# SerCharles/CN-RMA

Hardware: AMD Instinct MI355X
Metric: scenes/sec fwd (40-view->192^3 voxel): dense unprojection + RMA + voxelise + FCAF3D + decode (higher is better)
Workload: dtype f32 (sparse conv f16x3: 22-bit operands, fp32 accumulate; value_f32_conv = exact fp32); 1 GPU; NS: 40 views x 256 ch x 480x640 fp32 maps (channels_last) -> grid 192x192x192, N=300, max_points=500000, FCAF3D MinkResNet34 + head, 1 HIP graph per scene, 3 in flight; M_rows=72216505, M_selected=500000, M_unique=496819

## Files before the change

### cn-rma_amd/csrc/common.h

```cpp
#pragma once
#include <hip/hip_runtime.h>
#include <stdint.h>

#include "../../include/cnrma.h"

#define CNRMA_LAUNCH_CHECK()                      \
  do {                                            \
    hipError_t e__ = hipGetLastError();           \
    if (e__ != hipSuccess) return -(int)e__;      \
  } while (0)

static inline hipStream_t as_stream(void* s) { return reinterpret_cast<hipStream_t>(s); }
static inline int64_t ceil_div(int64_t a, int64_t b) { return (a + b - 1) / b; }

template <int UNUSED = 0>
__global__ __launch_bounds__(256) void cnrma_fill_kernel(uint32_t* __restrict__ p, uint32_t word, size_t n_words) {
  const size_t n4 = (((uintptr_t)p & 15) == 0) ? n_words / 4 : 0;
  const uint4 w4 = make_uint4(word, word, word, word);
  for (size_t i = (size_t)blockIdx.x * blockDim.x + threadIdx.x; i < n4; i += (size_t)gridDim.x * blockDim.x)
    reinterpret_cast<uint4*>(p)[i] = w4;
  for (size_t i = 4 * n4 + (size_t)blockIdx.x * blockDim.x + threadIdx.x; i < n_words; i += (size_t)gridDim.x * blockDim.x)
    p[i] = word;
}
static inline hipError_t cnrma_fill_bytes(void* p, int byte, size_t n_bytes, hipStream_t st) {
  if (n_bytes == 0) return hipSuccess;
  if ((n_bytes & 3) != 0 || ((uintptr_t)p & 3) != 0) return hipMemsetAsync(p, byte, n_bytes, st);
  const uint32_t b = (uint32_t)(byte & 0xFF), word = b | (b << 8) | (b << 16) | (b << 24);
  size_t blocks = (n_bytes / 16 + 255) / 256;
  blocks = blocks < 1 ? 1 : (blocks > 2048 ? 2048 : blocks);
  hipLaunchKernelGGL(cnrma_fill_kernel<0>, dim3((unsigned)blocks), dim3(256), 0, st, reinterpret_cast<uint32_t*>(p), word,
                     n_bytes / 4);
  return hipGetLastError();
}
// ... 139 lines not shown
```

### cn-rma_amd/csrc/sparse.hip

```cpp
#include <cstdio>
#include <type_traits>
#include "common.h"

#include <hipcub/hipcub.hpp>

namespace {

struct UniqueWs {
  int32_t* slot;
  int32_t* idx;
  uint8_t* flag;
  void* scan;
  uint64_t* key_a; uint64_t* key_b;
  int32_t* val_a; int32_t* val_b;
  void* sort_tmp; size_t sort_tmp_bytes;
  int32_t* range_err;
};

size_t sort_temp_bytes(int64_t n) {
  size_t bytes = 0;
  hipError_t e = hipcub::DeviceRadixSort::SortPairs(nullptr, bytes, (const uint64_t*)nullptr, (uint64_t*)nullptr,
                                                    (const int32_t*)nullptr, (int32_t*)nullptr, (int)n, 0, 64, nullptr);
  if (e != hipSuccess || bytes == 0) bytes = (size_t)n * 16 + (1u << 20);
  (void)hipGetLastError();
// ... 3275 lines not shown
                                               int64_t no_cap, int precleared, void* stream) {
  if (n_cap <= 0 || no_cap <= 0 || in_stride <= 0 || kernel_size < 1 || kernel_size > 3) return CNRMA_EINVAL;
  const int K = kernel_size * kernel_size * kernel_size;
  hipStream_t st = as_stream(stream);
  if (!precleared) {
    hipError_t e = cnrma_fill_bytes(nbr, 0xFF, (size_t)no_cap * K * sizeof(int32_t), st);
    if (e != hipSuccess) return -(int)e;
  }
  hipLaunchKernelGGL(kernel_map_strided_kernel, dim3((unsigned)ceil_div(n_cap, 256)), dim3(256), 0, st, in_coords,
                     n_cap, n_dev, in_stride, kernel_size, out_hash_keys, out_hash_vals, hash_cap, nbr);
  CNRMA_LAUNCH_CHECK();
  return 0;
}

extern "C" size_t cnrma_sparse_conv_workspace_bytes(int64_t no_cap, int Cout, int K) {
  if (K <= 1 || no_cap >= 65536) return 0;
  return (size_t)K * (size_t)no_cap * (size_t)Cout * sizeof(float);
}

#ifdef CNRMA_EXPERIMENTS
extern "C" int cnrma_debug_conv_tuning(const int* v, int n) {
  ConvTune t;
  int* f[] = {&t.shape, &t.splits, &t.pf, &t.ablate, &t.ws, &t.xcd, &t.go, &t.nb};
  if (n < 0 || n > 8 || (n > 0 && v == nullptr)) return CNRMA_EINVAL;
  for (int i = 0; i < n; ++i) *f[i] = v[i];
  g_conv_tune = t;
  return 0;
}
#endif

extern "C" int cnrma_sparse_conv_plan(int64_t no_cap, int Cin, int Cout, int K, int mode, int slices, size_t workspace_bytes,
                                      int* out6) {
  if (out6 == nullptr || Cin <= 0 || Cout <= 0 || K <= 0 || K > 27 || no_cap <= 0 || mode < 0 || mode > 3) return CNRMA_EINVAL;
  const bool six = mode != 0 && Cin % 32 == 0;
  const ConvMode m = mode == 3 ? CONV_EXACT : static_cast<ConvMode>(mode);
  const ConvPlan pl = plan_conv(no_cap, Cin, Cout, K, m, six, slices > 1 ? slices : 1, workspace_bytes > 0, workspace_bytes);
  out6[0] = pl.bm; out6[1] = pl.bn; out6[2] = pl.splits; out6[3] = pl.k_per_split; out6[4] = pl.pf; out6[5] = pl.shape;
  return 0;
}

extern "C" int cnrma_sparse_conv_f32(const float* in_feats, int Cin, const int32_t* nbr, int K, const float* weight,
                                     int Cout, const float* scale, const float* shift, const float* residual, int act,
                                     float* out_feats, int64_t no_cap, const int32_t* no_dev, void* workspace,
                                     size_t workspace_bytes, void* stream) {
  ConvArgs p = conv_args(in_feats, Cin, nbr, K, Cout, out_feats, no_cap, no_dev, workspace);
  p.weight = weight;
  return launch_conv(with_epilogue(p, scale, shift, residual, act), CONV_EXACT, nullptr, workspace_bytes, as_stream(stream));
}
// ... 977 lines not shown
```

### cn-rma_amd/csrc/util.hip

```cpp
#include "common.h"

extern "C" int cnrma_abi_version(void) { return CNRMA_ABI_VERSION; }

extern "C" int cnrma_fill_bytes_u8(void* dst, int byte, size_t n_bytes, void* stream) {
  if (dst == nullptr || (n_bytes & 3) != 0 || (reinterpret_cast<uintptr_t>(dst) & 3) != 0) return CNRMA_EINVAL;
  if (n_bytes == 0) return 0;
  const hipError_t e = cnrma_fill_bytes(dst, byte, n_bytes, reinterpret_cast<hipStream_t>(stream));
  return e == hipSuccess ? 0 : -(int)e;
}

__global__ __launch_bounds__(256) void range_violations_kernel(const int32_t* __restrict__ v, const int32_t* __restrict__ lo,
                                                               const int32_t* __restrict__ hi, int n, int32_t* __restrict__ out) {
  __shared__ int sm[4];
  int c = 0;
  for (int i = threadIdx.x; i < n; i += 256) c += (v[i] < lo[i] || v[i] > hi[i]) ? 1 : 0;
  for (int o = 32; o > 0; o >>= 1) c += __shfl_down(c, o, 64);
  if ((threadIdx.x & 63) == 0) sm[threadIdx.x >> 6] = c;
  __syncthreads();
  if (threadIdx.x == 0) out[0] = sm[0] + sm[1] + sm[2] + sm[3];
}

extern "C" int cnrma_range_violations_i32(const int32_t* values, const int32_t* lo, const int32_t* hi, int n, int32_t* out,
                                          void* stream) {
  if (values == nullptr || lo == nullptr || hi == nullptr || out == nullptr || n <= 0 || n > 4096) return CNRMA_EINVAL;
  hipLaunchKernelGGL(range_violations_kernel, dim3(1), dim3(256), 0, reinterpret_cast<hipStream_t>(stream), values, lo, hi, n, out);
  CNRMA_LAUNCH_CHECK();
  return 0;
}

namespace {

constexpr int SCAN_BLOCK = 256;
constexpr int SCAN_VECS = 4;
constexpr int SCAN_ITEMS = 4 * SCAN_VECS;
constexpr int SCAN_TILE = SCAN_BLOCK * SCAN_ITEMS;
constexpr int SCAN_WAVE_ITEMS = 64 * SCAN_ITEMS;

template <typename T>
__device__ __forceinline__ int scan_load(const T* in, int64_t i, int64_t n) {
  return i < n ? (int)in[i] : 0;
}

__device__ __forceinline__ int64_t scan_vec_base(int64_t tile_base, int k) {
  return tile_base + (int64_t)(threadIdx.x >> 6) * SCAN_WAVE_ITEMS + (int64_t)(k * 64 + (threadIdx.x & 63)) * 4;
}

template <typename T>
__device__ __forceinline__ void scan_load_vec(const T* __restrict__ in, int64_t i, int64_t n, bool wide, int v[4]) {
  static_assert(sizeof(T) == 4 || sizeof(T) == 1, "int32 items or byte masks");
  if (wide) {
    if constexpr (sizeof(T) == 4) {
      const int4 q = *reinterpret_cast<const int4*>(in + i);
      v[0] = q.x; v[1] = q.y; v[2] = q.z; v[3] = q.w;
    } else {
      const uint32_t q = *reinterpret_cast<const uint32_t*>(in + i);
      v[0] = (int)(q & 255u); v[1] = (int)((q >> 8) & 255u); v[2] = (int)((q >> 16) & 255u); v[3] = (int)(q >> 24);
    }
  } else {
#pragma unroll
    for (int j = 0; j < 4; ++j) v[j] = scan_load(in, i + j, n);
  }
}

template <typename T>
__global__ __launch_bounds__(SCAN_BLOCK) void scan_tile_sums(const T* __restrict__ in, int32_t* __restrict__ tile_sum,
                                                             int64_t n, int aligned) {
  __shared__ int smem[SCAN_BLOCK / 64 + 1];
  const int64_t tile_base = (int64_t)blockIdx.x * SCAN_TILE;
  const bool wide = aligned != 0 && tile_base + SCAN_TILE <= n;
  int s = 0;
#pragma unroll
  for (int k = 0; k < SCAN_VECS; ++k) {
    int v[4];
    scan_load_vec(in, scan_vec_base(tile_base, k), n, wide, v);
    s += (v[0] + v[1]) + (v[2] + v[3]);
  }
  int total;
  block_excl_scan<SCAN_BLOCK>(s, smem, &total);
  if (threadIdx.x == 0) tile_sum[blockIdx.x] = total;
}

__global__ __launch_bounds__(1024) void scan_tile_offsets(int32_t* __restrict__ tile_sum, int64_t n_tiles) {
  __shared__ int smem[1024 / 64 + 1];
  const int64_t per = (n_tiles + 1023) / 1024;
  const int64_t lo = (int64_t)threadIdx.x * per;
  const int64_t hi = lo + per < n_tiles ? lo + per : n_tiles;
  int s = 0;
  for (int64_t i = lo; i < hi; ++i) s += tile_sum[i];
  int total;
  int run = block_excl_scan<1024>(s, smem, &total);
  for (int64_t i = lo; i < hi; ++i) {
    const int v = tile_sum[i];
    tile_sum[i] = run;
    run += v;
  }
  if (threadIdx.x == 0) tile_sum[n_tiles] = total;
}

template <typename T, int MODE, bool OWN_OFFSET>
__global__ __launch_bounds__(SCAN_BLOCK) void scan_apply(const T* __restrict__ in, const int32_t* __restrict__ tile_off,
                                                         int32_t* __restrict__ out, int32_t* __restrict__ total_out,
                                                         int64_t n, int64_t n_tiles, int aligned) {
  __shared__ int smem[SCAN_BLOCK / 64 + 1];
  __shared__ int wave_sum[SCAN_BLOCK / 64];
  const int64_t tile_base = (int64_t)blockIdx.x * SCAN_TILE;
  const bool wide = aligned != 0 && tile_base + SCAN_TILE <= n;
  const int lane = threadIdx.x & 63, wid = threadIdx.x >> 6;
  int v[SCAN_VECS][4];
  int ex[SCAN_VECS];
  int run = 0;
#pragma unroll
  for (int k = 0; k < SCAN_VECS; ++k) {
    scan_load_vec(in, scan_vec_base(tile_base, k), n, wide, v[k]);
    const int q = (v[k][0] + v[k][1]) + (v[k][2] + v[k][3]);
    const int incl = wave_incl_scan(q);
    ex[k] = run + incl - q;
    run += __shfl(incl, 63, 64);
  }
  if (lane == 0) wave_sum[wid] = run;
  int offset, grand = 0;
  if constexpr (OWN_OFFSET) {
    const int upto = blockIdx.x == 0 ? (int)n_tiles : (int)blockIdx.x;
    int part = 0;
    for (int i = threadIdx.x; i < upto; i += SCAN_BLOCK) part += tile_off[i];
    int sum;
    block_excl_scan<SCAN_BLOCK>(part, smem, &sum);
    offset = blockIdx.x == 0 ? 0 : sum;
// ... 12 lines not shown
    int at = offset + ex[k];
#pragma unroll
    for (int j = 0; j < 4; ++j) {
      r[j] = (MODE == 0) ? at : (v[k][j] ? at : -1);
      at += v[k][j];
    }
    if (wide) {
      *reinterpret_cast<int4*>(out + i) = make_int4(r[0], r[1], r[2], r[3]);
    } else {
#pragma unroll
      for (int j = 0; j < 4; ++j)
        if (i + j < n) out[i + j] = r[j];
    }
  }
  if (blockIdx.x == 0 && threadIdx.x == 0) {
    if (MODE == 0) out[n] = grand;
    if (total_out) total_out[0] = grand;
  }
}

constexpr int SCAN_SINGLE_MAX = 32768;
template <typename T, int MODE>
__global__ __launch_bounds__(1024) void scan_single_kernel(const T* __restrict__ in, int32_t* __restrict__ out,
                                                           int32_t* __restrict__ total_out, int n) {
  __shared__ int smem[1024 / 64 + 1];
  const int per = (n + 1023) / 1024;
  const int lo = threadIdx.x * per, hi = min(lo + per, n);
  int s = 0;
  for (int i = lo; i < hi; ++i) s += (int)in[i];
  int total;
  int run = block_excl_scan<1024>(s, smem, &total);
  for (int i = lo; i < hi; ++i) {
    const int v = (int)in[i];
    out[i] = (MODE == 0) ? run : (v ? run : -1);
    run += v;
  }
  if (threadIdx.x == 0) {
    if (MODE == 0) out[n] = total;
    if (total_out) total_out[0] = total;
  }
}

template <typename T, int MODE>
int run_scan(const T* in, int32_t* out, int32_t* total_out, int64_t n, void* workspace, hipStream_t st) {
  if (n < 0) return CNRMA_EINVAL;
  if (n <= SCAN_SINGLE_MAX) {
    hipLaunchKernelGGL((scan_single_kernel<T, MODE>), dim3(1), dim3(1024), 0, st, in, out, total_out, (int)n);
    CNRMA_LAUNCH_CHECK();
    return 0;
  }
  int64_t n_tiles = ceil_div(n > 0 ? n : 1, SCAN_TILE);
  int32_t* tile = reinterpret_cast<int32_t*>(workspace);
  const int aligned = (reinterpret_cast<uintptr_t>(out) & 15) == 0 && (reinterpret_cast<uintptr_t>(in) & (4 * sizeof(T) - 1)) == 0;
  hipLaunchKernelGGL((scan_tile_sums<T>), dim3((unsigned)n_tiles), dim3(SCAN_BLOCK), 0, st, in, tile, n, aligned);
  if (n_tiles <= SCAN_TILE) {
    hipLaunchKernelGGL((scan_apply<T, MODE, true>), dim3((unsigned)n_tiles), dim3(SCAN_BLOCK), 0, st, in, tile, out, total_out,
                       n, n_tiles, aligned);
  } else {
    hipLaunchKernelGGL(scan_tile_offsets, dim3(1), dim3(1024), 0, st, tile, n_tiles);
    hipLaunchKernelGGL((scan_apply<T, MODE, false>), dim3((unsigned)n_tiles), dim3(SCAN_BLOCK), 0, st, in, tile, out, total_out,
                       n, n_tiles, aligned);
  }
  CNRMA_LAUNCH_CHECK();
  return 0;
}

__global__ __launch_bounds__(256) void sum_f64_partial(const double* __restrict__ in, double* __restrict__ part,
                                                       int64_t n) {
  __shared__ double sm[4];
  double s = 0.0;
  for (int64_t i = (int64_t)blockIdx.x * 256 + threadIdx.x; i < n; i += (int64_t)gridDim.x * 256) s += in[i];
#pragma unroll
  for (int d = 32; d > 0; d >>= 1) s += __shfl_down(s, d, 64);
  if ((threadIdx.x & 63) == 0) sm[threadIdx.x >> 6] = s;
  __syncthreads();
  if (threadIdx.x == 0) part[blockIdx.x] = (sm[0] + sm[1]) + (sm[2] + sm[3]);
}

__global__ __launch_bounds__(256) void sum_f64_final(const double* __restrict__ part, int nparts,
                                                     double* __restrict__ out) {
  __shared__ double sm[4];
  double s = 0.0;
  for (int i = threadIdx.x; i < nparts; i += 256) s += part[i];
#pragma unroll
// ... 96 lines not shown
    if (c0 + c < C && p0 + 8 * q < HW) v = *reinterpret_cast<const uint4*>(s + (int64_t)(c0 + c) * HW + p0 + 8 * q);
    const uint32_t w[4] = {v.x, v.y, v.z, v.w};
#pragma unroll
    for (int i = 0; i < 4; ++i) { tile[c][8 * q + 2 * i] = (uint16_t)(w[i] & 0xffffu); tile[c][8 * q + 2 * i + 1] = (uint16_t)(w[i] >> 16); }
  }
  __syncthreads();
#pragma unroll
  for (int j = 0; j < 2; ++j) {
    const int p = r + 32 * j;
    if (c0 + 8 * q < C && p0 + p < HW) {
      uint32_t w[4];
#pragma unroll
      for (int i = 0; i < 4; ++i) w[i] = (uint32_t)tile[8 * q + 2 * i][p] | ((uint32_t)tile[8 * q + 2 * i + 1][p] << 16);
      *reinterpret_cast<uint4*>(d + (p0 + p) * C + c0 + 8 * q) = make_uint4(w[0], w[1], w[2], w[3]);
    }
  }
}

__device__ __forceinline__ uint32_t row_hash(uint32_t seed, uint32_t i) {
  uint32_t x = i * 0x9E3779B1u + seed;
  x ^= x >> 16; x *= 0x7FEB352Du; x ^= x >> 15; x *= 0x846CA68Bu; x ^= x >> 16;
  return x;
}

__device__ __forceinline__ uint32_t select_key(const float* __restrict__ scores, uint32_t seed, uint32_t i) {
  if (scores == nullptr) return row_hash(seed, i);
  const uint32_t u = __float_as_uint(scores[i]);
  const uint32_t ordered = (u & 0x80000000u) ? ~u : (u | 0x80000000u);
  return ~ordered;
}

struct SampleWs {
  int32_t hist[3][2048];
  int32_t prefix[3];
  int32_t need[4];
  int32_t tie_count, pad;
  int32_t tie_idx[256];
  int32_t prefix2[3];
  int32_t pad3;
  int32_t list_count, pad2;
  uint64_t list[1024];
};
constexpr size_t SAMPLE_WS_ZEROED = offsetof(SampleWs, list);

__device__ __forceinline__ int key_digit(uint32_t k, int pass) {
  return pass == 0 ? (int)(k >> 21) : (pass == 1 ? (int)((k >> 10) & 2047u) : (int)(k & 1023u));
}
__device__ __forceinline__ bool key_matches(uint32_t k, int pass, const int32_t* prefix) {
  if (pass >= 1 && (int)(k >> 21) != prefix[0]) return false;
  if (pass >= 2 && (int)((k >> 10) & 2047u) != prefix[1]) return false;
  return true;
}

__device__ __forceinline__ void resolve_digit(const int32_t* __restrict__ hist, int need, int* digit, int* need_next,
                                              int* smem ) {
  int bins[8], local = 0;
#pragma unroll
  for (int j = 0; j < 8; ++j) { bins[j] = hist[8 * threadIdx.x + j]; local += bins[j]; }
  int* out = smem + 256 / 64 + 1;
  if (threadIdx.x == 0) { out[0] = 0; out[1] = 0; }
  int total;
  int ex = block_excl_scan<256>(local, smem, &total);
  if (ex < need && ex + local >= need) {
#pragma unroll
    for (int j = 0; j < 8; ++j) {
      if (ex < need && ex + bins[j] >= need) { out[0] = 8 * threadIdx.x + j; out[1] = need - ex; }
      ex += bins[j];
    }
  }
  __syncthreads();
  *digit = out[0];
  *need_next = out[1];
  __syncthreads();
}

__device__ __forceinline__ int64_t select_rows(const int32_t* __restrict__ m_dev, int64_t m_cap) {
  const int64_t m = m_dev[0];
  return m < m_cap ? m : m_cap;
}
__device__ __forceinline__ uint32_t select_seed(uint32_t seed, const uint32_t* __restrict__ seed_dev) {
  return seed_dev ? seed + 0x9E3779B9u * seed_dev[0] : seed;
}

__global__ __launch_bounds__(256) void sample_hist_kernel(const int32_t* __restrict__ m_dev, int64_t m_cap,
                                                          const float* __restrict__ scores, uint32_t seed,
                                                          const uint32_t* __restrict__ seed_dev, int pass, int n_keep,
                                                          SampleWs* __restrict__ ws) {
  seed = select_seed(seed, seed_dev);
  __shared__ int h[2048];
  __shared__ int rs[256 / 64 + 1 + 2];
  int32_t prefix[3] = {0, 0, 0};
  int need = n_keep;
  for (int q = 0; q < pass; ++q) {
    int nn;
    resolve_digit(ws->hist[q], need, &prefix[q], &nn, rs);
    need = nn;
  }
  for (int i = threadIdx.x; i < 2048; i += 256) h[i] = 0;
  __syncthreads();
  const int64_t M = select_rows(m_dev, m_cap);
  for (int64_t i = (int64_t)blockIdx.x * blockDim.x + threadIdx.x; i < M; i += (int64_t)gridDim.x * blockDim.x) {
    const uint32_t k = select_key(scores, seed, (uint32_t)i);
    if (key_matches(k, pass, prefix)) atomicAdd(&h[key_digit(k, pass)], 1);
  }
  __syncthreads();
  for (int i = threadIdx.x; i < 2048; i += 256)
    if (h[i]) atomicAdd(&ws->hist[pass][i], h[i]);
}

__global__ __launch_bounds__(256) void sample_ties_kernel(const int32_t* __restrict__ m_dev, int64_t m_cap,
                                                          const float* __restrict__ scores, uint32_t seed,
                                                          const uint32_t* __restrict__ seed_dev, int n_keep,
                                                          SampleWs* __restrict__ ws) {
  seed = select_seed(seed, seed_dev);
  __shared__ int rs[256 / 64 + 1 + 2];
  int32_t prefix[3];
  int need = n_keep;
  for (int q = 0; q < 3; ++q) {
    int nn;
    resolve_digit(ws->hist[q], need, &prefix[q], &nn, rs);
    need = nn;
  }
  if (blockIdx.x == 0 && threadIdx.x == 0) {
    ws->prefix[0] = prefix[0]; ws->prefix[1] = prefix[1]; ws->prefix[2] = prefix[2];
    ws->need[0] = n_keep; ws->need[3] = need;
  }
  const int64_t M = select_rows(m_dev, m_cap);
  const uint32_t key = ((uint32_t)prefix[0] << 21) | ((uint32_t)prefix[1] << 10) | (uint32_t)prefix[2];
  for (int64_t i = (int64_t)blockIdx.x * blockDim.x + threadIdx.x; i < M; i += (int64_t)gridDim.x * blockDim.x) {
    if (select_key(scores, seed, (uint32_t)i) == key) {
      const int slot = atomicAdd(&ws->tie_count, 1);
      if (slot < 256) ws->tie_idx[slot] = (int32_t)i;
    }
  }
}

__global__ __launch_bounds__(1024) void sample_tie_select_kernel(const int32_t* __restrict__ m_dev, int64_t m_cap,
                                                                const float* __restrict__ scores, uint32_t seed,
                                                                const uint32_t* __restrict__ seed_dev,
                                                                SampleWs* __restrict__ ws) {
  if (ws->tie_count <= 256) return;
  seed = select_seed(seed, seed_dev);
  __shared__ int h[2048];
  __shared__ int sh_digit, sh_need;
  const int64_t M = select_rows(m_dev, m_cap);
  const uint32_t key = ((uint32_t)ws->prefix[0] << 21) | ((uint32_t)ws->prefix[1] << 10) | (uint32_t)ws->prefix[2];
  int32_t prefix2[3] = {0, 0, 0};
  int need = ws->need[3];
  for (int pass = 0; pass < 3; ++pass) {
    for (int i = threadIdx.x; i < 2048; i += 1024) h[i] = 0;
    __syncthreads();
    for (int64_t i = threadIdx.x; i < M; i += 1024) {
      if (select_key(scores, seed, (uint32_t)i) != key) continue;
      const uint32_t k2 = (uint32_t)i;
      if (key_matches(k2, pass, prefix2)) atomicAdd(&h[key_digit(k2, pass)], 1);
    }
    __syncthreads();
    if (threadIdx.x == 0) {
      int cum = 0, d = 0, nn = 0;
      for (int bin = 0; bin < 2048; ++bin) {
        if (cum < need && cum + h[bin] >= need) { d = bin; nn = need - cum; break; }
        cum += h[bin];
      }
      sh_digit = d; sh_need = nn;
// ... 69 lines not shown
  const int t = threadIdx.x;
  const int n = min(min(ws->list_count, k), 1024);
  a[t] = t < n ? ws->list[t] : ~0ull;
  __syncthreads();
  for (int size = 2; size <= 1024; size <<= 1) {
    for (int stride = size >> 1; stride > 0; stride >>= 1) {
      const int partner = t ^ stride;
      if (partner > t) {
        const bool up = (t & size) == 0;
        const uint64_t x = a[t], y = a[partner];
        if ((x > y) == up) { a[t] = y; a[partner] = x; }
      }
      __syncthreads();
    }
  }
  if (t < k) out[t] = t < n ? (int64_t)(uint32_t)a[t] : 0;
}

__global__ __launch_bounds__(256) void select_count_segments_kernel(int64_t R, const int32_t* __restrict__ off,
                                                                    const int32_t* __restrict__ m_dev, int64_t m_cap,
                                                                    uint32_t seed, const uint32_t* __restrict__ seed_dev,
                                                                    const SampleWs* __restrict__ ws, int n_keep,
                                                                    int32_t* __restrict__ counts) {
  seed = select_seed(seed, seed_dev);
  const int64_t M = select_rows(m_dev, m_cap);
  __shared__ int32_t sh_bound;
  __shared__ int rs[256 / 64 + 1 + 2];
  const int32_t tie_bound = select_tie_bound(ws, &sh_bound, rs);
  const bool all = M <= n_keep;
  const uint32_t key = ((uint32_t)ws->prefix[0] << 21) | ((uint32_t)ws->prefix[1] << 10) | (uint32_t)ws->prefix[2];
  const int64_t r = (int64_t)blockIdx.x * blockDim.x + threadIdx.x;
  if (r >= R) return;
  int64_t m0 = off[r], m1 = off[r + 1];
  if (m1 > M) m1 = M;
  int c = 0;
  for (int64_t i = m0; i < m1; ++i) {
    const uint32_t k = row_hash(seed, (uint32_t)i);
    c += (all || k < key || (k == key && (int32_t)i <= tie_bound)) ? 1 : 0;
  }
  counts[r] = c;
}

__global__ __launch_bounds__(256) void select_scatter_records_kernel(int64_t R, const int32_t* __restrict__ off,
                                                                     const int32_t* __restrict__ sel_off,
                                                                     const int2* __restrict__ kept, int cap,
                                                                     const int32_t* __restrict__ m_dev, int64_t m_cap,
                                                                     uint32_t seed, const uint32_t* __restrict__ seed_dev,
                                                                     const SampleWs* __restrict__ ws, int n_keep,
                                                                     int64_t rec_cap, int4* __restrict__ rec) {
  seed = select_seed(seed, seed_dev);
  const int64_t M = select_rows(m_dev, m_cap);
  __shared__ int32_t sh_bound;
  __shared__ int rs[256 / 64 + 1 + 2];
  const int32_t tie_bound = select_tie_bound(ws, &sh_bound, rs);
  const bool all = M <= n_keep;
  const uint32_t key = ((uint32_t)ws->prefix[0] << 21) | ((uint32_t)ws->prefix[1] << 10) | (uint32_t)ws->prefix[2];
  const int64_t r = (int64_t)blockIdx.x * blockDim.x + threadIdx.x;
  if (r >= R) return;
  const int64_t m0 = off[r];
  int64_t m1 = off[r + 1];
  if (m1 > M) m1 = M;
  int64_t j = sel_off[r];
  for (int64_t i = m0; i < m1; ++i) {
    const uint32_t k = row_hash(seed, (uint32_t)i);
    if (all || k < key || (k == key && (int32_t)i <= tie_bound)) {
      if (j < rec_cap && i - m0 < cap) {
        const int2 kv = kept[r * cap + (i - m0)];
        rec[j] = make_int4((int)r, kv.y, kv.x, 0);
      }
      ++j;
    }
  }
}

}

extern "C" size_t cnrma_sample_workspace_bytes(void) { return sizeof(SampleWs); }

static int run_select(const int32_t* m_dev, const float* scores, int64_t m_cap, int n_keep, uint32_t seed,
                      const uint32_t* seed_dev, uint8_t* mask, void* workspace, hipStream_t st, int64_t* out_idx = nullptr) {
  if (m_cap <= 0 || n_keep <= 0 || m_cap >= ((int64_t)1 << 31)) return CNRMA_EINVAL;
  SampleWs* ws = reinterpret_cast<SampleWs*>(workspace);
  hipError_t e = cnrma_fill_bytes(ws, 0, SAMPLE_WS_ZEROED, st);
  if (e != hipSuccess) return -(int)e;
  int blocks = (int)(m_cap / 2048 + 1);
  if (blocks > 1024) blocks = 1024;
  for (int pass = 0; pass < 3; ++pass)
    hipLaunchKernelGGL(sample_hist_kernel, dim3(blocks), dim3(256), 0, st, m_dev, m_cap, scores, seed, seed_dev, pass,
                       n_keep, ws);
  hipLaunchKernelGGL(sample_ties_kernel, dim3(blocks), dim3(256), 0, st, m_dev, m_cap, scores, seed, seed_dev, n_keep, ws);
  hipLaunchKernelGGL(sample_tie_select_kernel, dim3(1), dim3(1024), 0, st, m_dev, m_cap, scores, seed, seed_dev, ws);
  if (mask != nullptr) {
    hipLaunchKernelGGL(sample_mask_kernel, dim3(blocks), dim3(256), 0, st, m_dev, m_cap, scores, seed, seed_dev, ws, n_keep,
                       mask);
  } else if (out_idx == nullptr) {
  } else {
    hipLaunchKernelGGL(sample_collect_kernel, dim3(blocks), dim3(256), 0, st, m_dev, m_cap, scores, ws, n_keep);
    hipLaunchKernelGGL(topk_sort_kernel, dim3(1), dim3(1024), 0, st, ws, n_keep, out_idx);
  }
  CNRMA_LAUNCH_CHECK();
  return 0;
}

extern "C" int cnrma_sample_mask(const int32_t* m_dev, int64_t m_cap, int n_keep, uint32_t seed, const uint32_t* seed_dev,
                                 uint8_t* mask, void* workspace, void* stream) {
  if (m_dev == nullptr) return CNRMA_EINVAL;
  return run_select(m_dev, nullptr, m_cap, n_keep, seed, seed_dev, mask, workspace, as_stream(stream));
}

extern "C" int cnrma_topk_mask_f32(const float* scores, const int32_t* n_dev, int64_t n_cap, int k, uint8_t* mask,
                                   void* workspace, void* stream) {
  if (scores == nullptr || n_dev == nullptr) return CNRMA_EINVAL;
  return run_select(n_dev, scores, n_cap, k, 0u, nullptr, mask, workspace, as_stream(stream));
}

extern "C" int cnrma_rma_select_records(const int32_t* row_offset, int64_t R, const void* kept, int cap, const int32_t* m_dev,
                                        int64_t m_cap, int n_keep, uint32_t seed, const uint32_t* seed_dev, void* sample_ws,
                                        int32_t* ray_counts, int32_t* ray_offsets, void* scan_ws, int64_t rec_cap,
                                        void* records, int32_t* n_sel, void* stream) {
  if (row_offset == nullptr || kept == nullptr || m_dev == nullptr || R <= 0 || cap <= 0 || records == nullptr ||
      ray_counts == nullptr || ray_offsets == nullptr || n_sel == nullptr)
    return CNRMA_EINVAL;
  hipStream_t st = as_stream(stream);
  int rc = run_select(m_dev, nullptr, m_cap, n_keep, seed, seed_dev, nullptr, sample_ws, st, nullptr);
  if (rc != 0) return rc;
  const SampleWs* ws = reinterpret_cast<const SampleWs*>(sample_ws);
  const unsigned blocks = (unsigned)ceil_div(R, 256);
  hipLaunchKernelGGL(select_count_segments_kernel, dim3(blocks), dim3(256), 0, st, R, row_offset, m_dev, m_cap, seed, seed_dev,
                     ws, n_keep, ray_counts);
  rc = run_scan<int32_t, 0>(ray_counts, ray_offsets, n_sel, R, scan_ws, st);
  if (rc != 0) return rc;
  hipLaunchKernelGGL(select_scatter_records_kernel, dim3(blocks), dim3(256), 0, st, R, row_offset, ray_offsets,
                     reinterpret_cast<const int2*>(kept), cap, m_dev, m_cap, seed, seed_dev, ws, n_keep, rec_cap,
                     reinterpret_cast<int4*>(records));
  CNRMA_LAUNCH_CHECK();
  return 0;
}

extern "C" int cnrma_topk_indices_f32(const float* scores, const int32_t* n_dev, int64_t n_cap, int k, int64_t* out_idx,
                                      void* workspace, void* stream) {
  if (scores == nullptr || n_dev == nullptr || out_idx == nullptr || k > 1024) return CNRMA_EINVAL;
  return run_select(n_dev, scores, n_cap, k, 0u, nullptr, nullptr, workspace, as_stream(stream), out_idx);
}

extern "C" size_t cnrma_scan_workspace_bytes(int64_t n) {
  int64_t n_tiles = ceil_div(n > 0 ? n : 1, SCAN_TILE);
  size_t scan = (size_t)(n_tiles + 2) * sizeof(int32_t);
  size_t sum = 1024 * sizeof(double);
  return (scan > sum ? scan : sum) + 64;
}

extern "C" int cnrma_exclusive_scan_i32(const int32_t* in, int32_t* out, int64_t n, void* workspace, void* stream) {
  return run_scan<int32_t, 0>(in, out, nullptr, n, workspace, as_stream(stream));
// ... 51 lines not shown
```

### include/cnrma.h

```cpp
#ifndef CNRMA_H
#define CNRMA_H

#include <stddef.h>
#include <stdint.h>

#ifdef __cplusplus
extern "C" {
#endif

#define CNRMA_EINVAL (-22)
#define CNRMA_ABI_VERSION 7

int cnrma_abi_version(void);

int cnrma_fill_bytes_u8(void* dst, int byte, size_t n_bytes, void* stream);

int cnrma_range_violations_i32(const int32_t* values, const int32_t* lo, const int32_t* hi, int n, int32_t* out, void* stream);

int cnrma_nchw_to_nhwc_f32(const float* feat_nchw, float* feat_nhwc, int V, int C, int H, int W, void* stream);

#define CNRMA_DENSE_WORKSPACE_BYTES 1024
#define CNRMA_DENSE_MASK_BYTES(X, Y, Z, V)                                                                              \
  ((((((int64_t)(X) + 31) / 32) * (((int64_t)(Y) + 31) / 32) * (((int64_t)(Z) + 31) / 32) + 7) * 512) *               \
   (((int64_t)(V) + 63) / 64) * 8)
// ... 63 lines not shown
                                 float* out_xyz, int xyz_stride, float* out_w, int w_stride, float* out_feat,
                                 int feat_stride, int32_t* out_sample, void* stream);
int cnrma_rma_neus_emit_rows_ref_f32(const float* proj_inv, const float* const* feat_nhwc_ref, int V, int C, int H, int W,
                                 int n_steps, float t_one, const int32_t* row_offset, int64_t n_out,
                                 const int32_t* n_out_dev, const void* kept, int cap, const int32_t* sel_index,
                                 int64_t sel_cap, void* records, const float* w_div, float addx, float addy, float addz,
                                 float* out_xyz, int xyz_stride, float* out_w, int w_stride, float* out_feat,
                                 int feat_stride, int32_t* out_sample, void* stream);
int cnrma_rma_neus_emit_rows_h16(const float* proj_inv, const void* feat_nhwc, const void* const* feat_nhwc_ref, int elem,
                                 int V, int C, int H, int W,
                                 int n_steps, float t_one, const int32_t* row_offset, int64_t n_out,
                                 const int32_t* n_out_dev, const void* kept, int cap, const int32_t* sel_index,
                                 int64_t sel_cap, void* records, const float* w_div, float addx, float addy, float addz,
                                 float* out_xyz, int xyz_stride, float* out_w, int w_stride, float* out_feat,
                                 int feat_stride, int32_t* out_sample, void* stream);

size_t cnrma_sample_workspace_bytes(void);
int cnrma_sample_mask(const int32_t* m_dev, int64_t m_cap, int n_keep, uint32_t seed, const uint32_t* seed_dev,
                      uint8_t* mask, void* workspace, void* stream);
int cnrma_rma_select_records(const int32_t* row_offset, int64_t R, const void* kept, int cap, const int32_t* m_dev,
                             int64_t m_cap, int n_keep, uint32_t seed, const uint32_t* seed_dev, void* sample_ws,
                             int32_t* ray_counts, int32_t* ray_offsets, void* scan_ws, int64_t rec_cap, void* records,
                             int32_t* n_sel, void* stream);
int cnrma_topk_mask_f32(const float* scores, const int32_t* n_dev, int64_t n_cap, int k, uint8_t* mask,
                        void* workspace, void* stream);
int cnrma_topk_indices_f32(const float* scores, const int32_t* n_dev, int64_t n_cap, int k, int64_t* out_idx,
                           void* workspace, void* stream);

int cnrma_rma_depth_count_f32(const float* proj_inv, const float* tsdf, int V, int H, int W, int X, int Y, int Z,
                              float voxel_size, float ox, float oy, float oz, int n_steps, float t_one,
                              int select_grids, int32_t* count, double* wsum, void* stream);

int cnrma_rma_depth_emit_f32(const float* proj_inv, const float* tsdf, const float* feat_nhwc, int V, int C, int H,
                             int W, int X, int Y, int Z, float voxel_size, float ox, float oy, float oz,
                             int n_steps, float t_one, int select_grids, const int32_t* row_offset,
                             const int32_t* sel_index, const float* w_div, float addx, float addy, float addz,
                             float* out_xyz, int xyz_stride, float* out_w, int w_stride, float* out_feat,
                             int feat_stride, int64_t sel_cap, int64_t out_cap, void* stream);

int cnrma_rma_drop_single_sample_views(int32_t* count, double* wsum, int V, int64_t rays_per_view, void* stream);

int cnrma_rma_mean_weight(const double* wsum_total, const int32_t* m_total, float* mean_w, void* stream);

size_t cnrma_scan_workspace_bytes(int64_t n);
int cnrma_exclusive_scan_i32(const int32_t* in, int32_t* out, int64_t n, void* workspace, void* stream);
int cnrma_sum_f64(const double* in, double* out, int64_t n, void* workspace, void* stream);
// ... 258 lines not shown
```

Baseline: 64.60 scenes/s.

## Select sampled rows by inverting the row hash instead of radix-selecting all rows

Adds a key-space selection path for the random row subsampling in RMA. Because the row hash is a bijection, its inverse maps the smallest hash keys straight back to row indices. The new path enumerates only a window slightly larger than the expected key threshold, counts live rows per chunk, ranks them, marks the chosen rows in a bitmap, scans the popcounts and places the records. This avoids the three radix-histogram passes over all ~72M rows and the per-ray count/scan/scatter. A device-side route flag gates the old kernels so they run only when the window holds too few rows, at the cost of extra launches and more code paths.

```diff
diff --git a/cn-rma_amd/csrc/common.h b/cn-rma_amd/csrc/common.h
--- a/cn-rma_amd/csrc/common.h
+++ b/cn-rma_amd/csrc/common.h
@@ -9,6 +9,10 @@
     hipError_t e__ = hipGetLastError();           \
     if (e__ != hipSuccess) return -(int)e__;      \
   } while (0)
+
+#ifdef CNRMA_EXPERIMENTS
+namespace cnrma_exp { int select_tuning(const int* v, int n); }
+#endif
 
 static inline hipStream_t as_stream(void* s) { return reinterpret_cast<hipStream_t>(s); }
 static inline int64_t ceil_div(int64_t a, int64_t b) { return (a + b - 1) / b; }
diff --git a/cn-rma_amd/csrc/sparse.hip b/cn-rma_amd/csrc/sparse.hip
--- a/cn-rma_amd/csrc/sparse.hip
+++ b/cn-rma_amd/csrc/sparse.hip
@@ -3321,8 +3321,10 @@
 extern "C" int cnrma_debug_conv_tuning(const int* v, int n) {
   ConvTune t;
   int* f[] = {&t.shape, &t.splits, &t.pf, &t.ablate, &t.ws, &t.xcd, &t.go, &t.nb};
-  if (n < 0 || n > 8 || (n > 0 && v == nullptr)) return CNRMA_EINVAL;
-  for (int i = 0; i < n; ++i) *f[i] = v[i];
+  if (n < 0 || n > 11 || (n > 0 && v == nullptr)) return CNRMA_EINVAL;
+  const int rc = cnrma_exp::select_tuning(n > 8 ? v + 8 : nullptr, n > 8 ? n - 8 : 0);
+  if (rc != 0) return rc;
+  for (int i = 0; i < n && i < 8; ++i) *f[i] = v[i];
   g_conv_tune = t;
   return 0;
 }
diff --git a/cn-rma_amd/csrc/util.hip b/cn-rma_amd/csrc/util.hip
--- a/cn-rma_amd/csrc/util.hip
+++ b/cn-rma_amd/csrc/util.hip
@@ -36,9 +36,24 @@
 constexpr int SCAN_TILE = SCAN_BLOCK * SCAN_ITEMS;
 constexpr int SCAN_WAVE_ITEMS = 64 * SCAN_ITEMS;
 
+struct BitWord {
+  uint32_t w;
+  __device__ __forceinline__ explicit operator int() const { return __popc(w); }
+};
+template <typename T>
+__device__ __forceinline__ int scan_item(int raw) {
+  if constexpr (__is_same(T, BitWord)) return __popc((uint32_t)raw);
+  else return raw;
+}
+
 template <typename T>
 __device__ __forceinline__ int scan_load(const T* in, int64_t i, int64_t n) {
   return i < n ? (int)in[i] : 0;
+}
+
+constexpr int32_t SCAN_GATE_KEY = 1;
+__device__ __forceinline__ bool scan_gated_off(const int32_t* __restrict__ gate, int want_key) {
+  return gate != nullptr && (gate[0] == SCAN_GATE_KEY) != (want_key != 0);
 }
 
 __device__ __forceinline__ int64_t scan_vec_base(int64_t tile_base, int k) {
@@ -51,7 +66,7 @@
   if (wide) {
     if constexpr (sizeof(T) == 4) {
       const int4 q = *reinterpret_cast<const int4*>(in + i);
-      v[0] = q.x; v[1] = q.y; v[2] = q.z; v[3] = q.w;
+      v[0] = scan_item<T>(q.x); v[1] = scan_item<T>(q.y); v[2] = scan_item<T>(q.z); v[3] = scan_item<T>(q.w);
     } else {
       const uint32_t q = *reinterpret_cast<const uint32_t*>(in + i);
       v[0] = (int)(q & 255u); v[1] = (int)((q >> 8) & 255u); v[2] = (int)((q >> 16) & 255u); v[3] = (int)(q >> 24);
@@ -64,8 +79,10 @@
 
 template <typename T>
 __global__ __launch_bounds__(SCAN_BLOCK) void scan_tile_sums(const T* __restrict__ in, int32_t* __restrict__ tile_sum,
-                                                             int64_t n, int aligned) {
+                                                             int64_t n, int aligned, const int32_t* __restrict__ gate,
+                                                             int want_key) {
   __shared__ int smem[SCAN_BLOCK / 64 + 1];
+  if (scan_gated_off(gate, want_key)) return;
   const int64_t tile_base = (int64_t)blockIdx.x * SCAN_TILE;
   const bool wide = aligned != 0 && tile_base + SCAN_TILE <= n;
   int s = 0;
@@ -80,8 +97,10 @@
   if (threadIdx.x == 0) tile_sum[blockIdx.x] = total;
 }
 
-__global__ __launch_bounds__(1024) void scan_tile_offsets(int32_t* __restrict__ tile_sum, int64_t n_tiles) {
+__global__ __launch_bounds__(1024) void scan_tile_offsets(int32_t* __restrict__ tile_sum, int64_t n_tiles,
+                                                          const int32_t* __restrict__ gate, int want_key) {
   __shared__ int smem[1024 / 64 + 1];
+  if (scan_gated_off(gate, want_key)) return;
   const int64_t per = (n_tiles + 1023) / 1024;
   const int64_t lo = (int64_t)threadIdx.x * per;
   const int64_t hi = lo + per < n_tiles ? lo + per : n_tiles;
@@ -100,9 +119,11 @@
 template <typename T, int MODE, bool OWN_OFFSET>
 __global__ __launch_bounds__(SCAN_BLOCK) void scan_apply(const T* __restrict__ in, const int32_t* __restrict__ tile_off,
                                                          int32_t* __restrict__ out, int32_t* __restrict__ total_out,
-                                                         int64_t n, int64_t n_tiles, int aligned) {
+                                                         int64_t n, int64_t n_tiles, int aligned,
+                                                         const int32_t* __restrict__ gate, int want_key) {
   __shared__ int smem[SCAN_BLOCK / 64 + 1];
   __shared__ int wave_sum[SCAN_BLOCK / 64];
+  if (scan_gated_off(gate, want_key)) return;
   const int64_t tile_base = (int64_t)blockIdx.x * SCAN_TILE;
   const bool wide = aligned != 0 && tile_base + SCAN_TILE <= n;
   const int lane = threadIdx.x & 63, wid = threadIdx.x >> 6;
@@ -161,8 +182,10 @@
 constexpr int SCAN_SINGLE_MAX = 32768;
 template <typename T, int MODE>
 __global__ __launch_bounds__(1024) void scan_single_kernel(const T* __restrict__ in, int32_t* __restrict__ out,
-                                                           int32_t* __restrict__ total_out, int n) {
+                                                           int32_t* __restrict__ total_out, int n,
+                                                           const int32_t* __restrict__ gate, int want_key) {
   __shared__ int smem[1024 / 64 + 1];
+  if (scan_gated_off(gate, want_key)) return;
   const int per = (n + 1023) / 1024;
   const int lo = threadIdx.x * per, hi = min(lo + per, n);
   int s = 0;
@@ -181,24 +204,25 @@
 }
 
 template <typename T, int MODE>
-int run_scan(const T* in, int32_t* out, int32_t* total_out, int64_t n, void* workspace, hipStream_t st) {
+int run_scan(const T* in, int32_t* out, int32_t* total_out, int64_t n, void* workspace, hipStream_t st,
+             const int32_t* gate = nullptr, int want_key = 0) {
   if (n < 0) return CNRMA_EINVAL;
   if (n <= SCAN_SINGLE_MAX) {
-    hipLaunchKernelGGL((scan_single_kernel<T, MODE>), dim3(1), dim3(1024), 0, st, in, out, total_out, (int)n);
+    hipLaunchKernelGGL((scan_single_kernel<T, MODE>), dim3(1), dim3(1024), 0, st, in, out, total_out, (int)n, gate, want_key);
     CNRMA_LAUNCH_CHECK();
     return 0;
   }
   int64_t n_tiles = ceil_div(n > 0 ? n : 1, SCAN_TILE);
   int32_t* tile = reinterpret_cast<int32_t*>(workspace);
   const int aligned = (reinterpret_cast<uintptr_t>(out) & 15) == 0 && (reinterpret_cast<uintptr_t>(in) & (4 * sizeof(T) - 1)) == 0;
-  hipLaunchKernelGGL((scan_tile_sums<T>), dim3((unsigned)n_tiles), dim3(SCAN_BLOCK), 0, st, in, tile, n, aligned);
+  hipLaunchKernelGGL((scan_tile_sums<T>), dim3((unsigned)n_tiles), dim3(SCAN_BLOCK), 0, st, in, tile, n, aligned, gate, want_key);
   if (n_tiles <= SCAN_TILE) {
     hipLaunchKernelGGL((scan_apply<T, MODE, true>), dim3((unsigned)n_tiles), dim3(SCAN_BLOCK), 0, st, in, tile, out, total_out,
-                       n, n_tiles, aligned);
+                       n, n_tiles, aligned, gate, want_key);
   } else {
-    hipLaunchKernelGGL(scan_tile_offsets, dim3(1), dim3(1024), 0, st, tile, n_tiles);
+    hipLaunchKernelGGL(scan_tile_offsets, dim3(1), dim3(1024), 0, st, tile, n_tiles, gate, want_key);
     hipLaunchKernelGGL((scan_apply<T, MODE, false>), dim3((unsigned)n_tiles), dim3(SCAN_BLOCK), 0, st, in, tile, out, total_out,
-                       n, n_tiles, aligned);
+                       n, n_tiles, aligned, gate, want_key);
   }
   CNRMA_LAUNCH_CHECK();
   return 0;
@@ -341,6 +365,11 @@
   x ^= x >> 16; x *= 0x7FEB352Du; x ^= x >> 15; x *= 0x846CA68Bu; x ^= x >> 16;
   return x;
 }
+__device__ __forceinline__ uint32_t row_hash_inv(uint32_t seed, uint32_t k) {
+  uint32_t x = k;
+  x ^= x >> 16; x *= 0x43021123u; x ^= (x >> 15) ^ (x >> 30); x *= 0x1D69E2A5u; x ^= x >> 16;
+  return (x - seed) * 0x0E8B2F51u;
+}
 
 __device__ __forceinline__ uint32_t select_key(const float* __restrict__ scores, uint32_t seed, uint32_t i) {
   if (scores == nullptr) return row_hash(seed, i);
@@ -353,7 +382,8 @@
   int32_t hist[3][2048];
   int32_t prefix[3];
   int32_t need[4];
-  int32_t tie_count, pad;
+  int32_t tie_count;
+  int32_t route;
   int32_t tie_idx[256];
   int32_t prefix2[3];
   int32_t pad3;
@@ -361,6 +391,7 @@
   uint64_t list[1024];
 };
 constexpr size_t SAMPLE_WS_ZEROED = offsetof(SampleWs, list);
+constexpr int32_t SELECT_ROUTE_KEY = SCAN_GATE_KEY, SELECT_ROUTE_ROW_FALLBACK = 2;
 
 __device__ __forceinline__ int key_digit(uint32_t k, int pass) {
   return pass == 0 ? (int)(k >> 21) : (pass == 1 ? (int)((k >> 10) & 2047u) : (int)(k & 1023u));
@@ -405,6 +436,7 @@
                                                           const float* __restrict__ scores, uint32_t seed,
                                                           const uint32_t* __restrict__ seed_dev, int pass, int n_keep,
                                                           SampleWs* __restrict__ ws) {
+  if (ws->route == SELECT_ROUTE_KEY) return;
   seed = select_seed(seed, seed_dev);
   __shared__ int h[2048];
   __shared__ int rs[256 / 64 + 1 + 2];
@@ -431,6 +463,7 @@
                                                           const float* __restrict__ scores, uint32_t seed,
                                                           const uint32_t* __restrict__ seed_dev, int n_keep,
                                                           SampleWs* __restrict__ ws) {
+  if (ws->route == SELECT_ROUTE_KEY) return;
   seed = select_seed(seed, seed_dev);
   __shared__ int rs[256 / 64 + 1 + 2];
   int32_t prefix[3];
@@ -458,7 +491,7 @@
                                                                 const float* __restrict__ scores, uint32_t seed,
                                                                 const uint32_t* __restrict__ seed_dev,
                                                                 SampleWs* __restrict__ ws) {
-  if (ws->tie_count <= 256) return;
+  if (ws->tie_count <= 256 || ws->route == SELECT_ROUTE_KEY) return;
   seed = select_seed(seed, seed_dev);
   __shared__ int h[2048];
   __shared__ int sh_digit, sh_need;
@@ -574,6 +607,7 @@
                                                                     uint32_t seed, const uint32_t* __restrict__ seed_dev,
                                                                     const SampleWs* __restrict__ ws, int n_keep,
                                                                     int32_t* __restrict__ counts) {
+  if (ws->route == SELECT_ROUTE_KEY) return;
   seed = select_seed(seed, seed_dev);
   const int64_t M = select_rows(m_dev, m_cap);
   __shared__ int32_t sh_bound;
@@ -600,6 +634,7 @@
                                                                      uint32_t seed, const uint32_t* __restrict__ seed_dev,
                                                                      const SampleWs* __restrict__ ws, int n_keep,
                                                                      int64_t rec_cap, int4* __restrict__ rec) {
+  if (ws->route == SELECT_ROUTE_KEY) return;
   seed = select_seed(seed, seed_dev);
   const int64_t M = select_rows(m_dev, m_cap);
   __shared__ int32_t sh_bound;
@@ -625,16 +660,183 @@
   }
 }
 
-}
+struct KeyPlan {
+  uint32_t window16, window_add;
+  uint32_t chunk_keys, n_chunks;
+  uint64_t k_lim;
+};
+
+__device__ __forceinline__ uint64_t select_key_window(int64_t M, int n_keep, const KeyPlan& p) {
+  if (M <= n_keep) return 0;
+  const uint64_t t = ((uint64_t)n_keep << 32) / (uint64_t)M;
+  const uint64_t k0 = t * p.window16 / 16 + p.window_add;
+  return k0 < (1ull << 32) ? k0 : (1ull << 32);
+}
+
+__global__ __launch_bounds__(256) void select_key_count_kernel(const int32_t* __restrict__ m_dev, int64_t m_cap, uint32_t seed,
+                                                               const uint32_t* __restrict__ seed_dev, int n_keep, KeyPlan p,
+                                                               int32_t* __restrict__ chunk_count,
+                                                               uint32_t* __restrict__ bitmap, int64_t n_words) {
+  seed = select_seed(seed, seed_dev);
+  for (int64_t w = (int64_t)blockIdx.x * 256 + threadIdx.x; w < n_words; w += (int64_t)gridDim.x * 256) bitmap[w] = 0u;
+  const uint32_t chunk = blockIdx.x * 4u + (threadIdx.x >> 6), lane = threadIdx.x & 63u;
+  if (chunk >= p.n_chunks) return;
+  const int64_t M = select_rows(m_dev, m_cap);
+  const uint64_t K0 = select_key_window(M, n_keep, p);
+  const uint64_t k_lo = (uint64_t)chunk * p.chunk_keys;
+  uint64_t k_hi = k_lo + p.chunk_keys;
+  if (k_hi > K0) k_hi = K0;
+  if (K0 > p.k_lim) k_hi = 0;
+  int c = 0;
+  for (uint64_t base = k_lo; base < k_hi; base += 64) {
+    const uint64_t k = base + lane;
+    const bool live = k < k_hi && row_hash_inv(seed, (uint32_t)k) < (uint32_t)M;
+    c += __popcll(__ballot(live));
+  }
+  if (lane == 0) chunk_count[chunk] = c;
+}
+
+__global__ __launch_bounds__(1024) void select_key_resolve_kernel(const int32_t* __restrict__ m_dev, int64_t m_cap, int n_keep,
+                                                                  KeyPlan p, int32_t* __restrict__ chunk_count,
+                                                                  SampleWs* __restrict__ ws) {
+  __shared__ int smem[1024 / 64 + 1];
+  const int n = (int)p.n_chunks, per = (n + 1023) / 1024;
+  const int lo = min((int)threadIdx.x * per, n), hi = min(lo + per, n);
+  int s = 0;
+  for (int i = lo; i < hi; ++i) s += chunk_count[i];
+  int total;
+  int run = block_excl_scan<1024>(s, smem, &total);
+  for (int i = lo; i < hi; ++i) {
+    const int v = chunk_count[i];
+    chunk_count[i] = run;
+    run += v;
+  }
+  if (threadIdx.x == 0) {
+    const uint64_t K0 = select_key_window(select_rows(m_dev, m_cap), n_keep, p);
+    ws->route = (K0 > 0 && K0 <= p.k_lim && total >= n_keep) ? SELECT_ROUTE_KEY : SELECT_ROUTE_ROW_FALLBACK;
+  }
+}
+
+__global__ __launch_bounds__(256) void select_key_mark_kernel(const int32_t* __restrict__ m_dev, int64_t m_cap, uint32_t seed,
+                                                              const uint32_t* __restrict__ seed_dev, int n_keep, KeyPlan p,
+                                                              const int32_t* __restrict__ chunk_prefix,
+                                                              const SampleWs* __restrict__ ws, int64_t R,
+                                                              const int32_t* __restrict__ off, uint32_t* __restrict__ bitmap) {
+  if (ws->route != SELECT_ROUTE_KEY) return;
+  seed = select_seed(seed, seed_dev);
+  const uint32_t chunk = blockIdx.x * 4u + (threadIdx.x >> 6), lane = threadIdx.x & 63u;
+  if (chunk >= p.n_chunks) return;
+  int rank = chunk_prefix[chunk];
+  if (rank >= n_keep) return;
+  const int64_t M = select_rows(m_dev, m_cap);
+  const uint64_t K0 = select_key_window(M, n_keep, p);
+  const uint64_t k_lo = (uint64_t)chunk * p.chunk_keys;
+  uint64_t k_hi = k_lo + p.chunk_keys;
+  if (k_hi > K0) k_hi = K0;
+  const int64_t row_lo = off[0], row_hi = off[R];
+  for (uint64_t base = k_lo; base < k_hi && rank < n_keep; base += 64) {
+    const uint64_t k = base + lane;
+    const uint32_t i = row_hash_inv(seed, (uint32_t)k);
+    const bool live = k < k_hi && i < (uint32_t)M;
+    const uint64_t b = __ballot(live);
+    const int mine = rank + __popcll(b & ((1ull << lane) - 1ull));
+    if (live && mine < n_keep && (int64_t)i >= row_lo && (int64_t)i < row_hi) atomicOr(&bitmap[i >> 5], 1u << (i & 31u));
+    rank += __popcll(b);
+  }
+}
+
+__global__ __launch_bounds__(256) void select_key_place_kernel(const SampleWs* __restrict__ ws, const uint32_t* __restrict__ bitmap,
+                                                               const int32_t* __restrict__ prefix, int64_t n_words, int64_t R,
+                                                               const int32_t* __restrict__ off, const int2* __restrict__ kept,
+                                                               int cap, int64_t rec_cap, int4* __restrict__ rec) {
+  if (ws->route != SELECT_ROUTE_KEY) return;
+  const int64_t w = (int64_t)blockIdx.x * 256 + threadIdx.x;
+  if (w >= n_words) return;
+  uint32_t bits = bitmap[w];
+  if (bits == 0u) return;
+  int64_t j = prefix[w];
+  int64_t r = 0;
+  while (bits != 0u) {
+    const int64_t i = w * 32 + __builtin_ctz(bits);
+    bits &= bits - 1u;
+    if (i >= off[r + 1]) {
+      int64_t lo = r + 1, hi = R - 1;
+      while (lo < hi) {
+        const int64_t mid = (lo + hi) >> 1;
+        if (off[mid + 1] > i) hi = mid; else lo = mid + 1;
+      }
+      r = lo;
+    }
+    const int64_t c = i - off[r];
+    if (j < rec_cap && c < cap) {
+      const int2 kv = kept[r * cap + c];
+      rec[j] = make_int4((int)r, kv.y, kv.x, 0);
+    }
+    ++j;
+  }
+}
+
+constexpr uint32_t SELECT_WINDOW16 = 17, SELECT_WINDOW_ADD = 65536;
+constexpr uint64_t SELECT_KEY_C_NUM = 2, SELECT_KEY_C_DEN = 3;
+constexpr uint32_t SELECT_CHUNK_KEYS = 4096, SELECT_MAX_CHUNKS = 65536;
+
+struct SelectTune { int route = -1; int window16 = (int)SELECT_WINDOW16; int window_add = (int)SELECT_WINDOW_ADD; };
+#ifdef CNRMA_EXPERIMENTS
+SelectTune g_select_tune;
+#define CNRMA_SELECT_TUNE g_select_tune
+#else
+constexpr SelectTune k_select_tune{};
+#define CNRMA_SELECT_TUNE k_select_tune
+#endif
+
+bool select_key_plan(int64_t m_cap, int n_keep, int64_t R, KeyPlan* p) {
+  const SelectTune t = CNRMA_SELECT_TUNE;
+  if (t.route == 0 || m_cap <= n_keep || ceil_div(m_cap, 32) > R) return false;
+  const unsigned __int128 lhs = (unsigned __int128)m_cap * (uint64_t)m_cap * SELECT_KEY_C_DEN;
+  const unsigned __int128 rhs = ((unsigned __int128)n_keep << 32) * SELECT_KEY_C_NUM;
+  if (t.route != 1 && lhs < rhs) return false;
+  p->window16 = (uint32_t)t.window16;
+  p->window_add = (uint32_t)t.window_add;
+  const uint64_t t_cap = ((uint64_t)n_keep << 32) / (uint64_t)m_cap;
+  uint64_t k_lim = 2 * (t_cap * p->window16 / 16 + p->window_add);
+  if (k_lim > (1ull << 32)) k_lim = 1ull << 32;
+  const uint64_t max_chunks = R < (int64_t)SELECT_MAX_CHUNKS ? (uint64_t)R : SELECT_MAX_CHUNKS;
+  uint64_t chunk = (k_lim + max_chunks - 1) / max_chunks;
+  chunk = (chunk + 63) / 64 * 64;
+  if (chunk < SELECT_CHUNK_KEYS) chunk = SELECT_CHUNK_KEYS;
+  p->chunk_keys = (uint32_t)chunk;
+  p->n_chunks = (uint32_t)((k_lim + chunk - 1) / chunk);
+  p->k_lim = (uint64_t)p->n_chunks * chunk;
+  return true;
+}
+
+}
+
+static_assert(offsetof(SampleWs, route) == sizeof(int32_t) * CNRMA_SAMPLE_WS_ROUTE_WORD, "include/cnrma.h names the route word");
+
+#ifdef CNRMA_EXPERIMENTS
+int cnrma_exp::select_tuning(const int* v, int n) {
+  SelectTune t;
+  int* f[] = {&t.route, &t.window16, &t.window_add};
+  if (n < 0 || n > 3 || (n > 0 && v == nullptr)) return CNRMA_EINVAL;
+  for (int i = 0; i < n; ++i) *f[i] = v[i];
+  if (t.route < -1 || t.route > 1 || t.window16 < 1 || t.window16 > 256 || t.window_add < 0) return CNRMA_EINVAL;
+  g_select_tune = t;
+  return 0;
+}
+#endif
 
 extern "C" size_t cnrma_sample_workspace_bytes(void) { return sizeof(SampleWs); }
 
 static int run_select(const int32_t* m_dev, const float* scores, int64_t m_cap, int n_keep, uint32_t seed,
-                      const uint32_t* seed_dev, uint8_t* mask, void* workspace, hipStream_t st, int64_t* out_idx = nullptr) {
+                      const uint32_t* seed_dev, uint8_t* mask, void* workspace, hipStream_t st, int64_t* out_idx = nullptr,
+                      bool cleared = false ) {
   if (m_cap <= 0 || n_keep <= 0 || m_cap >= ((int64_t)1 << 31)) return CNRMA_EINVAL;
   SampleWs* ws = reinterpret_cast<SampleWs*>(workspace);
-  hipError_t e = cnrma_fill_bytes(ws, 0, SAMPLE_WS_ZEROED, st);
-  if (e != hipSuccess) return -(int)e;
+  if (!cleared) {
+    hipError_t e = cnrma_fill_bytes(ws, 0, SAMPLE_WS_ZEROED, st);
+    if (e != hipSuccess) return -(int)e;
+  }
   int blocks = (int)(m_cap / 2048 + 1);
   if (blocks > 1024) blocks = 1024;
   for (int pass = 0; pass < 3; ++pass)
@@ -673,14 +875,35 @@
   if (row_offset == nullptr || kept == nullptr || m_dev == nullptr || R <= 0 || cap <= 0 || records == nullptr ||
       ray_counts == nullptr || ray_offsets == nullptr || n_sel == nullptr)
     return CNRMA_EINVAL;
+  if (m_cap <= 0 || n_keep <= 0 || m_cap >= ((int64_t)1 << 31) || sample_ws == nullptr) return CNRMA_EINVAL;
   hipStream_t st = as_stream(stream);
-  int rc = run_select(m_dev, nullptr, m_cap, n_keep, seed, seed_dev, nullptr, sample_ws, st, nullptr);
+  SampleWs* ws = reinterpret_cast<SampleWs*>(sample_ws);
+  hipError_t e = cnrma_fill_bytes(ws, 0, SAMPLE_WS_ZEROED, st);
+  if (e != hipSuccess) return -(int)e;
+  KeyPlan plan;
+  const bool key = select_key_plan(m_cap, n_keep, R, &plan);
+  const int32_t* gate = key ? &ws->route : nullptr;
+  if (key) {
+    const int64_t n_words = ceil_div(m_cap, 32);
+    uint32_t* bitmap = reinterpret_cast<uint32_t*>(ray_counts);
+    const unsigned wave_blocks = (unsigned)ceil_div(plan.n_chunks, 4);
+    hipLaunchKernelGGL(select_key_count_kernel, dim3(wave_blocks), dim3(256), 0, st, m_dev, m_cap, seed, seed_dev, n_keep, plan,
+                       ray_offsets, bitmap, n_words);
+    hipLaunchKernelGGL(select_key_resolve_kernel, dim3(1), dim3(1024), 0, st, m_dev, m_cap, n_keep, plan, ray_offsets, ws);
+    hipLaunchKernelGGL(select_key_mark_kernel, dim3(wave_blocks), dim3(256), 0, st, m_dev, m_cap, seed, seed_dev, n_keep, plan,
+                       ray_offsets, ws, R, row_offset, bitmap);
+    int rk = run_scan<BitWord, 0>(reinterpret_cast<const BitWord*>(bitmap), ray_offsets, n_sel, n_words, scan_ws, st, gate, 1);
+    if (rk != 0) return rk;
+    hipLaunchKernelGGL(select_key_place_kernel, dim3((unsigned)ceil_div(n_words, 256)), dim3(256), 0, st, ws, bitmap,
+                       ray_offsets, n_words, R, row_offset, reinterpret_cast<const int2*>(kept), cap, rec_cap,
+                       reinterpret_cast<int4*>(records));
+  }
+  int rc = run_select(m_dev, nullptr, m_cap, n_keep, seed, seed_dev, nullptr, sample_ws, st, nullptr, true);
   if (rc != 0) return rc;
-  const SampleWs* ws = reinterpret_cast<const SampleWs*>(sample_ws);
   const unsigned blocks = (unsigned)ceil_div(R, 256);
   hipLaunchKernelGGL(select_count_segments_kernel, dim3(blocks), dim3(256), 0, st, R, row_offset, m_dev, m_cap, seed, seed_dev,
                      ws, n_keep, ray_counts);
-  rc = run_scan<int32_t, 0>(ray_counts, ray_offsets, n_sel, R, scan_ws, st);
+  rc = run_scan<int32_t, 0>(ray_counts, ray_offsets, n_sel, R, scan_ws, st, gate, 0);
   if (rc != 0) return rc;
   hipLaunchKernelGGL(select_scatter_records_kernel, dim3(blocks), dim3(256), 0, st, R, row_offset, ray_offsets,
                      reinterpret_cast<const int2*>(kept), cap, m_dev, m_cap, seed, seed_dev, ws, n_keep, rec_cap,
diff --git a/include/cnrma.h b/include/cnrma.h
--- a/include/cnrma.h
+++ b/include/cnrma.h
@@ -109,6 +109,7 @@
                              int64_t m_cap, int n_keep, uint32_t seed, const uint32_t* seed_dev, void* sample_ws,
                              int32_t* ray_counts, int32_t* ray_offsets, void* scan_ws, int64_t rec_cap, void* records,
                              int32_t* n_sel, void* stream);
+#define CNRMA_SAMPLE_WS_ROUTE_WORD 6152
 int cnrma_topk_mask_f32(const float* scores, const int32_t* n_dev, int64_t n_cap, int k, uint8_t* mask,
                         void* workspace, void* stream);
 int cnrma_topk_indices_f32(const float* scores, const int32_t* n_dev, int64_t n_cap, int k, int64_t* out_idx,
```

Result: no change. 65.06 scenes/s, median of 6 (+0.7%).
